# fanzhongyi/ExploreMultiModal

Hardware: AMD Instinct MI355X
Metric: image-text pairs/sec fwd+bwd, VLMo-Base, 1/2/4/8 MI355X; % bf16 MFMA roofline (higher is better)
Workload: dtype bf16

## Files before the change

exploremultimodal_amd/csrc/gemm_tn.hip:

```cpp
#include "gemm_common.h"
#include <algorithm>
#include <vector>

namespace {

struct GemmTN {
    const void* A;
    const void* B;
    float* C;
    int M, N1, N2, lda, ldb, ldc;
    int kt_per_split, tiles;
    float alpha;
    float* slab;
    int mode;
};
enum { TN_ATOMIC = 0, TN_ACCUM = 1, TN_STORE = 2 };

__device__ __attribute__((aligned(256))) char tn_zero_page[256];

__device__ __forceinline__ int tn_swz(int row) { return ((row & 3) << 2) | ((row >> 2) & 3); }

template <typename T, int BM, int BN, int WM, int WN, bool PP = false>
__device__ __forceinline__ void gemm_tn_body(const GemmTN& p, const int lid) {
    typedef typename Elem<T>::v8 v8;
    typedef typename Elem<T>::v4 v4;
    constexpr int NW = WM * WN;
    constexpr int SROWS = PP ? 32 : 64;
    constexpr int SUB = SROWS * 256;
    constexpr int NSA = BM / 128, NSB = BN / 128;
    constexpr int A_BYTES = NSA * SUB, STAGE = (NSA + NSB) * SUB;
    constexpr int TM = BM / WM / 32, TN = BN / WN / 32;
    constexpr int IPS = SROWS / 4;
    constexpr int IA = NSA * IPS / NW, IB = NSB * IPS / NW;
    static_assert((NSA * IPS) % NW == 0 && (NSB * IPS) % NW == 0, "tile/wave mismatch");
    static_assert(!PP || IA + IB == 4, "slice ring: four DMA instructions per wave and slice");
    extern __shared__ __attribute__((aligned(16))) char smem[];
    const int tid = threadIdx.x, lane = tid & 63;
    const int wave = __builtin_amdgcn_readfirstlane(tid >> 6);
    const int wm = wave / WN, wn = wave % WN;
    const int tiles_n = (p.N2 + BN - 1) / BN;
    const int split = lid / p.tiles, tile = lid - split * p.tiles;
    const int n1_0 = (tile / tiles_n) * BM, n2_0 = (tile % tiles_n) * BN;
    const int nk_total = (p.M + 63) >> 6;
    const int kt0 = split * p.kt_per_split;
    const int kt1 = min(nk_total, kt0 + p.kt_per_split);
    if (kt0 >= kt1) return;

// ... 184 lines not shown
                for (int r = 0; r < 16; ++r) {
                    const int gm = gm0 + (r & 3) + 8 * (r >> 2);
                    if (okn && gm < p.N1) p.C[(size_t)gm * p.ldc + gn] = old[r] + p.alpha * acc[i][j][r];
                }
            }
        return;
    }
#pragma unroll
    for (int i = 0; i < TM; ++i)
#pragma unroll
        for (int j = 0; j < TN; ++j) {
            const int gn = n2_0 + wn * (BN / WN) + j * 32 + l31;
#pragma unroll
            for (int r = 0; r < 16; ++r) {
                const int gm = n1_0 + wm * (BM / WM) + i * 32 + (r & 3) + 8 * (r >> 2) + 4 * h;
                if (gm < p.N1 && gn < p.N2) {
                    float* c = p.C + (size_t)gm * p.ldc + gn;
                    if (p.slab)
                        p.slab[((size_t)split * p.N1 + gm) * p.N2 + gn] = acc[i][j][r];
                    else if (p.mode == TN_STORE)
                        *c = p.alpha * acc[i][j][r];
                    else
                        atomicAdd(c, p.alpha * acc[i][j][r]);
                }
            }
        }
}

template <typename T, int BM, int BN, int WM, int WN, bool PP = false>
__global__ __launch_bounds__(WM * WN * 64, 2) void gemm_tn_kernel(const GemmTN p) {
    gemm_tn_body<T, BM, BN, WM, WN, PP>(p, xcd_remap(blockIdx.x, gridDim.x));
}

constexpr int MAX_TN_PROBS = 16;
constexpr int MAX_TN_ORDER = 1024;
constexpr uint16_t TN_NOP = 0xFFFF;
struct GemmTNMulti {
    int n;
    GemmTN p[MAX_TN_PROBS];
    uint16_t order[MAX_TN_ORDER];
};
template <typename T>
__global__ __launch_bounds__(512, 2) void gemm_tn_multi_kernel(const GemmTNMulti mp) {
    const uint32_t code = mp.order[blockIdx.x];
    if (code == TN_NOP) return;
    int gi = (int)(code >> 12);
    const int lid_in = __builtin_amdgcn_readfirstlane((int)(code & 0xFFFu));
    gi = __builtin_amdgcn_readfirstlane(gi);
    const GemmTN& q = mp.p[gi];
    GemmTN p;
    p.A = uniform_ptr(q.A), p.B = uniform_ptr(q.B), p.C = (float*)uniform_ptr(q.C);
    p.M = __builtin_amdgcn_readfirstlane(q.M), p.N1 = __builtin_amdgcn_readfirstlane(q.N1);
    p.N2 = __builtin_amdgcn_readfirstlane(q.N2), p.lda = __builtin_amdgcn_readfirstlane(q.lda);
    p.ldb = __builtin_amdgcn_readfirstlane(q.ldb), p.ldc = __builtin_amdgcn_readfirstlane(q.ldc);
    p.kt_per_split = __builtin_amdgcn_readfirstlane(q.kt_per_split), p.tiles = __builtin_amdgcn_readfirstlane(q.tiles);
    p.alpha = __builtin_bit_cast(float, __builtin_amdgcn_readfirstlane(__builtin_bit_cast(int, q.alpha)));
    p.slab = nullptr;
    p.mode = __builtin_amdgcn_readfirstlane(q.mode);
    gemm_tn_body<T, 256, 256, 2, 4, true>(p, lid_in);
}

__global__ __launch_bounds__(256) void tn_reduce_kernel(const float* __restrict__ slab, int splits, int N1, int N2,
                                                        float* __restrict__ C, int ldc, float alpha) {
    const int n4 = N2 >> 2;
    const long total = (long)N1 * n4;
    for (long i = (long)blockIdx.x * 256 + threadIdx.x; i < total; i += (long)gridDim.x * 256) {
        const int r = (int)(i / n4), c = (int)(i % n4) * 4;
        f32x4 a = {0.f, 0.f, 0.f, 0.f};
        for (int s2 = 0; s2 < splits; ++s2) a += *(const f32x4*)(slab + ((size_t)s2 * N1 + r) * N2 + c);
        f32x4* o = (f32x4*)(C + (size_t)r * ldc + c);
        *o = *o + alpha * a;
    }
}

struct TnPlan {
    int big, tiles, splits, per;
};
TnPlan tn_plan(int M, int N1, int N2, int splits_req, int force_tile) {
    const int nk = (M + 63) / 64;
    TnPlan pl{};
    const int t256 = ((N1 + 255) / 256) * ((N2 + 255) / 256);
    const int t128 = ((N1 + 127) / 128) * ((N2 + 127) / 128);
    const bool big_ok = N1 >= 256 && N2 >= 256 && nk >= 16 && t256 <= 256;
    pl.big = force_tile == 256 ? 1 : (force_tile == 128 ? 0 : (big_ok && (256 / t256) <= 16 && (256 / t256) >= 1 && nk / (256 / t256) >= 8));
    pl.tiles = pl.big ? t256 : t128;
    int splits = splits_req;
    if (splits <= 0) {
        if (pl.big) {
            splits = 256 / pl.tiles;
        } else {
            splits = 512 / pl.tiles;
            if (splits < 4) splits = 1024 / pl.tiles;
// ... 28 lines not shown
    }
    const TnPlan pl = tn_plan(M, N1, N2, splits, force);
    const bool use_slab = ws && pl.splits > 1 && N2 % 4 == 0 && ldc % 4 == 0 && ws_bytes >= (int64_t)pl.splits * N1 * N2 * 4;
    GemmTN p{A, B, C, M, N1, N2, lda, ldb, ldc, pl.per, pl.tiles, alpha, use_slab ? ws : nullptr, TN_ATOMIC};
    dim3 grid(pl.tiles * pl.splits);
    ProfScope prof(64 + (pl.big ? 8 : 0), 2.0 * M * N1 * N2, stream);
    if (pl.big) {
        constexpr int LDS = 2 * 4 * 64 * 256;
        static DeviceOnce attr;
        if (attr.first()) {
            (void)hipFuncSetAttribute((const void*)gemm_tn_kernel<bf16, 256, 256, 2, 4, true>, hipFuncAttributeMaxDynamicSharedMemorySize, LDS);
            (void)hipFuncSetAttribute((const void*)gemm_tn_kernel<f16, 256, 256, 2, 4, true>, hipFuncAttributeMaxDynamicSharedMemorySize, LDS);
        }
        if (dtype == VLMO_F16)
            hipLaunchKernelGGL((gemm_tn_kernel<f16, 256, 256, 2, 4, true>), grid, dim3(512), LDS, stream, p);
        else
            hipLaunchKernelGGL((gemm_tn_kernel<bf16, 256, 256, 2, 4, true>), grid, dim3(512), LDS, stream, p);
    } else {
        if (dtype == VLMO_F16)
            hipLaunchKernelGGL((gemm_tn_kernel<f16, 128, 128, 2, 2>), grid, dim3(256), 65536, stream, p);
        else
            hipLaunchKernelGGL((gemm_tn_kernel<bf16, 128, 128, 2, 2>), grid, dim3(256), 65536, stream, p);
    }
    VLMO_CHECK_LAUNCH("vlmo_gemm_tn");
    if (use_slab) {
        const long total = (long)N1 * (N2 / 4);
        const int rg = (int)((total + 255) / 256 < 2048 ? (total + 255) / 256 : 2048);
        hipLaunchKernelGGL(tn_reduce_kernel, dim3(rg), dim3(256), 0, stream, ws, pl.splits, N1, N2, C, ldc, alpha);
        VLMO_CHECK_LAUNCH("vlmo_gemm_tn(reduce)");
    }
    return 0;
}

extern "C" int vlmo_gemm_tn_multi(int dtype, const VlmoTnProblem* probs, int n, hipStream_t stream) {
    VLMO_CHECK_ARG(probs && n >= 1, "vlmo_gemm_tn_multi: no problems");
    VLMO_CHECK_ARG(dtype == VLMO_BF16 || dtype == VLMO_F16, "vlmo_gemm_tn_multi: dtype must be bf16 or f16");
    static DeviceOnce attr;
    if (attr.first()) {
        constexpr int LDS = 2 * 4 * 64 * 256;
        (void)hipFuncSetAttribute((const void*)gemm_tn_multi_kernel<bf16>, hipFuncAttributeMaxDynamicSharedMemorySize, LDS);
        (void)hipFuncSetAttribute((const void*)gemm_tn_multi_kernel<f16>, hipFuncAttributeMaxDynamicSharedMemorySize, LDS);
    }
    for (int q0 = 0, nq = 0; q0 < n; q0 += nq) {
        nq = 0;
        for (long tl = 0; q0 + nq < n && nq < MAX_TN_PROBS; ++nq) {
            const VlmoTnProblem& r = probs[q0 + nq];
            const long t = (long)((r.N1 + 255) / 256) * ((r.N2 + 255) / 256);
            if (nq > 0 && tl + t > MAX_TN_ORDER - 64) break;
            tl += t;
        }
        long tiles_all = 0;
        int min_nk = 1 << 30;
        double flops = 0;
        for (int q = 0; q < nq; ++q) {
            const VlmoTnProblem& r = probs[q0 + q];
            VLMO_CHECK_ARG(r.A && r.B && r.C, "vlmo_gemm_tn_multi: null operand in problem %d", q0 + q);
            VLMO_CHECK_ARG(r.M > 0 && r.N1 >= 8 && r.N2 >= 8 && r.N1 % 8 == 0 && r.N2 % 8 == 0 && r.lda % 8 == 0 &&
                               r.ldb % 8 == 0 && r.lda >= r.N1 && r.ldb >= r.N2 && r.ldc >= r.N2,
                           "vlmo_gemm_tn_multi: bad shape in problem %d (M=%d N1=%d N2=%d)", q0 + q, r.M, r.N1, r.N2);
            tiles_all += (long)((r.N1 + 255) / 256) * ((r.N2 + 255) / 256);
            const int nk = (r.M + 63) / 64;
            if (nk < min_nk) min_nk = nk;
            flops += 2.0 * r.M * r.N1 * r.N2;
        }
        int splits = 1;
        if (tiles_all < 192) {
            splits = (int)(256 / tiles_all);
            if (splits > min_nk / 8) splits = min_nk / 8;
            if (splits < 1) splits = 1;
        }
        GemmTNMulti mp{};
        mp.n = nq;
        struct Job {
            uint16_t code;
            int cost;
        };
        std::vector<Job> jobs;
        for (int q = 0; q < nq; ++q) {
            const VlmoTnProblem& r = probs[q0 + q];
            const int tiles = ((r.N1 + 255) / 256) * ((r.N2 + 255) / 256);
            const int nk = (r.M + 63) / 64;
            int sp = splits > nk ? nk : splits;
            const int per = (nk + sp - 1) / sp;
            sp = (nk + per - 1) / per;
            int mode = r.accumulate ? TN_ACCUM : TN_STORE;
            if (sp > 1) {
                mode = TN_ATOMIC;
                if (!r.accumulate) {
                    hipError_t rc = hipMemset2DAsync(r.C, (size_t)r.ldc * 4, 0, (size_t)r.N2 * 4, r.N1, stream);
                    if (rc != hipSuccess) {
                        vlmo_set_error("vlmo_gemm_tn_multi: memset failed: %s", hipGetErrorString(rc));
                        return (int)rc;
                    }
                }
            }
            VLMO_CHECK_ARG(tiles * sp <= 4096, "vlmo_gemm_tn_multi: problem %d has too many tiles", q0 + q);
            mp.p[q] = GemmTN{r.A, r.B, r.C, r.M, r.N1, r.N2, r.lda, r.ldb, r.ldc, per, tiles, r.alpha, nullptr, mode};
            for (int l = 0; l < tiles * sp; ++l) jobs.push_back(Job{(uint16_t)((q << 12) | l), per});
        }
        std::stable_sort(jobs.begin(), jobs.end(), [](const Job& a, const Job& b) { return a.cost > b.cost; });
        std::vector<uint16_t> bins[8];
        for (size_t i = 0; i < jobs.size();) {
            size_t j = i;
            while (j < jobs.size() && jobs[j].cost == jobs[i].cost) ++j;
            const size_t cnt = j - i;
            for (int x = 0; x < 8; ++x)
                for (size_t k = i + cnt * x / 8; k < i + cnt * (x + 1) / 8; ++k) bins[x].push_back(jobs[k].code);
            i = j;
        }
        size_t deepest = 0;
        for (int x = 0; x < 8; ++x) deepest = bins[x].size() > deepest ? bins[x].size() : deepest;
        VLMO_CHECK_ARG(deepest * 8 <= (size_t)MAX_TN_ORDER, "vlmo_gemm_tn_multi: %zu workgroups exceed one launch (pass fewer problems per call)",
                       jobs.size());
        const int t = (int)deepest * 8;
        for (int b = 0; b < t; ++b) {
            const std::vector<uint16_t>& bin = bins[b & 7];
            mp.order[b] = (size_t)(b >> 3) < bin.size() ? bin[b >> 3] : TN_NOP;
        }
        ProfScope prof(73, flops, stream);
        constexpr int LDS = 2 * 4 * 64 * 256;
        if (dtype == VLMO_F16)
            hipLaunchKernelGGL((gemm_tn_multi_kernel<f16>), dim3(t), dim3(512), LDS, stream, mp);
        else
            hipLaunchKernelGGL((gemm_tn_multi_kernel<bf16>), dim3(t), dim3(512), LDS, stream, mp);
        VLMO_CHECK_LAUNCH("vlmo_gemm_tn_multi");
    }
    return 0;
}
```

exploremultimodal_amd/hip.py:

```python
import ctypes
import os

import torch

_HERE = os.path.dirname(os.path.abspath(__file__))
LIB_PATH = os.environ.get('VLMO_HIP_LIB') or os.path.join(_HERE, 'lib', 'libvlmo_hip.so')

BF16, F16, F32 = 0, 1, 2
EPI_BIAS, EPI_BIAS_GELU, EPI_RESID, EPI_DGELU, EPI_F32, EPI_DUAL, EPI_ARGMAX, EPI_CE, EPI_CE_BWD = 0, 1, 2, 3, 4, 5, 6, 7, 8

_vp, _i32, _u32, _u64, _f32, _i64 = (ctypes.c_void_p, ctypes.c_int32, ctypes.c_uint32,
                                     ctypes.c_uint64, ctypes.c_float, ctypes.c_int64)


class Epilogue(ctypes.Structure):
    _fields_ = [('out', _vp), ('out2', _vp), ('bias', _vp), ('gamma', _vp),
                ('resid', _vp), ('row_scale', _vp), ('row_index', _vp), ('aux', _vp),
                ('ldo', _i32), ('ld2', _i32), ('relu', _i32),
                ('drop_thresh', _u32), ('inv_keep', _f32), ('beta', _f32),
                ('seed', _u64), ('colpart', _vp)]


_fp = _vp

# ... 49 lines not shown
                     ctypes.POINTER(Epilogue), _vp],
    'vlmo_gemm_tn': [_i32, _vp, _i32, _vp, _i32, _vp, _i32, _i32, _i32, _i32, _f32, _i32, _vp, _i64, _vp],
    'vlmo_ln_fwd': [_vp, _vp, _vp, _vp, _i32, _vp, _vp, _vp, _i32, _i32, _f32, _vp],
    'vlmo_ln_bwd': [_vp, _i32, _vp, _vp, _vp, _vp, _vp, _vp, _vp, _vp, _vp, _i32, _i32, _vp, _i64, _vp],
    'vlmo_ln_resid_bwd': [_vp, _vp, _vp, _vp, _vp, _vp, _vp, _vp, _vp, _vp, _vp, _vp, _vp, _vp, _vp, _vp, _u32, _f32, _u64,
                          _i32, _i32, _vp, _i64, _vp],
    'vlmo_attn_fwd': [_vp, _vp, _i32, _vp, _vp, _vp, _i32, _i32, _i32, _i32, _f32, _u32, _f32,
                      _u64, _i32, _vp],
    'vlmo_attn_bwd': [_vp, _vp, _vp, _vp, _i32, _vp, _i32, _vp, _vp, _vp, _i32, _i32, _i32, _f32,
                      _u32, _f32, _u64, _i32, _vp],
    'vlmo_resid_bwd': [_vp, _vp, _vp, _vp, _vp, _vp, _vp, _vp, _i32, _i32, _u32, _f32, _u64, _vp, _i64, _vp],
    'vlmo_colsum': [_i32, _vp, _i32, _vp, _i32, _i32, _vp, _i64, _vp],
    'vlmo_cast_weight': [_i32, _vp, _i32, _i32, _vp, _vp, _vp],
    'vlmo_cast_weight_multi': [_i32, _i32, _vp, _vp, _vp, _vp, _vp, _vp],
    'vlmo_patchify': [_vp, _vp, _i32, _i32, _i32, _i32, _i32, _vp],
    'vlmo_embed_img_finish': [_vp, _vp, _vp, _vp, _vp, _vp, _vp, _i32, _i32, _i32, _u32, _f32,
                              _u64, _vp],
    'vlmo_embed_img_bwd': [_vp, _vp, _vp, _vp, _vp, _vp, _vp, _i32, _i32, _i32, _u32, _f32,
                           _u64, _vp],
    'vlmo_embed_txt_fwd': [_vp] * 10 + [_i32, _i32, _i32, _f32, _u32, _f32, _u64, _vp],
    'vlmo_embed_txt_bwd': [_vp] * 11 + [_i32, _i32, _i32, _u32, _f32, _u64, _vp],
    'vlmo_conv2d_nhwc': [_i32, _i32, _vp, _i32, _i32, _i32, _i32, _i32, _vp, _i32, _vp,
                         ctypes.POINTER(Epilogue), _vp],
    'vlmo_dvae_im2col': [_vp, _vp, _i32, _i32, _i32, _i32, _i32, _i32, _vp],
    'vlmo_maxpool2_nhwc': [_vp, _vp, _vp, _i32, _i32, _i32, _i32, _vp],
    'vlmo_argmax_reduce': [_vp, _i32, _vp, _i32, _vp],
    'vlmo_dvae_embed': [_vp, _vp, _vp, _vp, _i32, _i32, _i32, _vp],
    'vlmo_upsample2_nhwc': [_vp, _vp, _i32, _i32, _i32, _i32, _vp],
    'vlmo_dvae_out_head': [_vp, _vp, _vp, _vp, _i32, _i32, _i32, _i32, _i32, _vp],
    'vlmo_ce_reduce': [_vp, _i32, _vp, _i32, _vp, _vp, _vp, _i32, _vp],
    'vlmo_stack_fwd': [ctypes.POINTER(StackDesc), _vp],
    'vlmo_stack_bwd': [ctypes.POINTER(StackDesc), _vp],
    'vlmo_gemm_tn_multi': [_i32, ctypes.POINTER(TnProblem), _i32, _vp],
    'vlmo_colwork_multi': [_i32, ctypes.POINTER(ColJob), _i32, _vp],
    'vlmo_event_create': [ctypes.POINTER(ctypes.c_void_p)],
    'vlmo_event_destroy': [_vp],
    'vlmo_stream_wait_event': [_vp, _vp],
    'vlmo_profile_start': [_i32],
    'vlmo_gemm_nt_grouped': [_i32, _i32, _i32, _i32, _vp, _i32, _vp, _i32, _vp, _i32, _i32, _vp, _vp],
    'vlmo_mt_grad_norm': [ctypes.c_void_p, _f32, _f32, _vp, _vp, _vp],
    'vlmo_mt_adam': [ctypes.c_void_p, ctypes.c_void_p, _vp, _vp],
    'vlmo_mt_ema': [ctypes.c_void_p, _f32, _vp],
    'vlmo_mt_adam_ema': [ctypes.c_void_p, ctypes.c_void_p, _vp, _vp, _f32, _vp],
    'vlmo_side_stream_create': [_i32, ctypes.POINTER(ctypes.c_uint32), _i32, ctypes.POINTER(ctypes.c_void_p)],
    'vlmo_profile_stop': [_i32, ctypes.POINTER(ctypes.c_double), ctypes.POINTER(ctypes.c_double),
                          ctypes.POINTER(ctypes.c_int64)],
    'vlmo_gemm_nt_2src': [_i32, _i32, _i32, _vp, _i32, _i32, _f32, _vp, _i32, _vp, _i32, _i32, _i32, _i32,
                          ctypes.POINTER(Epilogue), _vp],
    'vlmo_comm_available': [],
    'vlmo_comm_unique_id': [_vp],
    'vlmo_comm_init': [ctypes.POINTER(ctypes.c_void_p), _vp, _i32, _i32],
    'vlmo_comm_destroy': [_vp],
    'vlmo_comm_count': [_vp, _vp, _vp],
    'vlmo_comm_all_reduce': [_vp, _vp, _vp, _i64, _i32, _vp],
    'vlmo_comm_reduce_scatter': [_vp, _vp, _vp, _i64, _i32, _vp],
    'vlmo_comm_all_gather': [_vp, _vp, _vp, _i64, _i32, _vp],
    'vlmo_grad_pack': [_vp, _vp, _i64, _f32, _vp],
    'vlmo_grad_unpack': [_vp, _vp, _i64, _vp],
    'vlmo_ln_gelu_fwd': [_vp, _i32, _vp, _vp, _vp, _i32, _vp, _vp, _i32, _i32, _f32, _vp],
    'vlmo_ln_gelu_bwd': [_vp, _i32, _vp, _i32, _vp, _vp, _vp, _vp, _vp, _i32, _vp, _i32, _vp, _vp, _vp, _i32, _i32, _vp,
                         _i64, _vp],
    'vlmo_vqa_bce': [_vp, _i32, _vp, _i32, _i32, _i32, _vp, _vp, _vp, _vp, _f32, _vp, _i32, _vp, _i32, _vp],
    'vlmo_isda_update': [_vp, _i32, _vp, _vp, _vp, _vp, _vp, _i32, _i32, _i32, _i32, _vp, _vp, _vp, _vp, _vp],
    'vlmo_isda_aug_fwd': [_vp, _i32, _vp, _vp, _i32, _i32, _i32, _i32, _f32, _vp, _i32, _vp, _i64, _vp],
    'vlmo_isda_aug_bwd': [_vp, _i32, _vp, _i32, _vp, _vp, _i32, _i32, _i32, _i32, _f32, _vp, _i32, _vp, _i64, _vp],
    'vlmo_sim_topk': [_vp, _i32, _vp, _i32, _i32, _i32, _i32, _i32, _f32, _i32, _vp, ctypes.c_size_t, _vp, _vp, _vp],
# ... 265 lines not shown


def maxpool2_nhwc(x, raw, relu, B, H, W, C):
    _check(lib().vlmo_maxpool2_nhwc(_p(x), _p(raw), _p(relu), B, H, W, C, _stream()), 'vlmo_maxpool2_nhwc')


def argmax_reduce(partial, nchunk, ids, M):
    _check(lib().vlmo_argmax_reduce(_p(partial), nchunk, _p(ids), M, _stream()), 'vlmo_argmax_reduce')


def dvae_embed(ids, table, bias, out):
    vocab, n_init = table.shape
    _check(lib().vlmo_dvae_embed(_p(ids), _p(table), _p(bias), _p(out), ids.numel(), vocab, n_init, _stream()),
           'vlmo_dvae_embed')


def upsample2_nhwc(x, out, B, H, W, C):
    _check(lib().vlmo_upsample2_nhwc(_p(x), _p(out), B, H, W, C, _stream()), 'vlmo_upsample2_nhwc')


def dvae_out_head(x, w, bias, out, B, H, W):
    Cout, C = w.shape
    _check(lib().vlmo_dvae_out_head(_p(x), _p(w), _p(bias), _p(out), B, H, W, C, Cout, _stream()), 'vlmo_dvae_out_head')


def gemm_tn_multi(problems, dtype=BF16):
    n = len(problems)
    arr = (TnProblem * n)()
    for i, (A, B, C, M, N1, N2, acc) in enumerate(problems):
        arr[i] = TnProblem(_p(A), _p(B), _p(C), A.stride(0), B.stride(0), C.stride(0), M, N1, N2, 1.0, int(acc))
    _check(lib().vlmo_gemm_tn_multi(dtype, arr, n, _stream()), 'vlmo_gemm_tn_multi')


def colwork_multi(jobs, dtype=BF16):
    n = len(jobs)
    arr = (ColJob * n)()
    for i, (kind, src, rows, ncols, outs, n0) in enumerate(jobs):
        o = (ctypes.c_void_p * 4)(*[_p(t) for t in (list(outs) + [None] * 4)[:4]])
        arr[i] = ColJob(kind, src.stride(0), _p(src), rows, ncols, o, n0, 0)
    _check(lib().vlmo_colwork_multi(dtype, arr, n, _stream()), 'vlmo_colwork_multi')


def event_create():
    out = ctypes.c_void_p()
    _check(lib().vlmo_event_create(ctypes.byref(out)), 'vlmo_event_create')
    return out.value


def stream_wait_event(stream, ev):
    raw = stream.cuda_stream if hasattr(stream, 'cuda_stream') else stream
    _check(lib().vlmo_stream_wait_event(raw, ev), 'vlmo_stream_wait_event')


COMM_ID_BYTES = 128


def comm_available():
    return bool(lib().vlmo_comm_available())


def comm_unique_id():
    buf = ctypes.create_string_buffer(COMM_ID_BYTES)
    _check(lib().vlmo_comm_unique_id(buf), 'vlmo_comm_unique_id')
    return buf.raw


# ... 243 lines not shown
```

include/vlmo_hip.h:

```cpp
#ifndef VLMO_HIP_H
#define VLMO_HIP_H

#include <stddef.h>
#include <stdint.h>

#ifdef __cplusplus
extern "C" {
#endif

#ifndef __HIP_PLATFORM_AMD__
typedef struct ihipStream_t* hipStream_t;
#endif

enum { VLMO_BF16 = 0, VLMO_F16 = 1, VLMO_F32 = 2 };

enum {
    VLMO_EPI_BIAS = 0,
    VLMO_EPI_BIAS_GELU = 1,
    VLMO_EPI_RESID = 2,
    VLMO_EPI_DGELU = 3,
    VLMO_EPI_F32 = 4,
    VLMO_EPI_DUAL = 5,
    VLMO_EPI_ARGMAX = 6,
    VLMO_EPI_CE = 7,
// ... 16 lines not shown
    float beta;
    uint64_t seed;
    float* colpart;
} VlmoEpilogue;

const char* vlmo_last_error(void);
#define VLMO_ABI_VERSION 9
int vlmo_abi_version(void);

int vlmo_gemm_nt(int epi, int dtype, int tile, const void* A, int lda, const void* B, int ldb,
                 int M, int N, int K, const VlmoEpilogue* e, hipStream_t stream);
int vlmo_gemm_nt_2src(int epi, int dtype, int tile, const void* A, int lda, int k1, float seg_scale, const void* A2,
                      int lda2, const void* B, int ldb, int M, int N, int K, const VlmoEpilogue* e,
                      hipStream_t stream);
int vlmo_gemm_nt_grouped(int epi, int dtype, int tile, int ngroups, const void* const* A, int lda,
                         const void* const* B, int ldb, const int32_t* M, int N, int K,
                         const VlmoEpilogue* e, hipStream_t stream);

int64_t vlmo_gemm_tn_ws_bytes(int M, int N1, int N2);
int vlmo_gemm_tn(int dtype, const void* A, int lda, const void* B, int ldb, float* C, int ldc,
                 int M, int N1, int N2, float alpha, int splits, float* ws, int64_t ws_bytes,
                 hipStream_t stream);

typedef struct VlmoTnProblem {
    const void* A;
    const void* B;
    float* C;
    int32_t lda, ldb, ldc;
    int32_t M, N1, N2;
    float alpha;
    int32_t accumulate;
} VlmoTnProblem;
int vlmo_gemm_tn_multi(int dtype, const VlmoTnProblem* probs, int n, hipStream_t stream);

int vlmo_ln_fwd(const float* x, const float* w, const float* b, void* y, int out_f32,
                float* mean, float* rstd, const int32_t* rowmap, int M, int d, float eps,
                hipStream_t stream);
int64_t vlmo_reduce_ws_bytes(int ncols);

int vlmo_ln_bwd(const void* dy, int dy_f32, const int32_t* rowmap, const float* x, const float* w,
                const float* mean, const float* rstd, const float* dres, float* dx, float* dw,
                float* db, int M, int d, float* ws, int64_t ws_bytes, hipStream_t stream);

int vlmo_ln_resid_bwd(const void* dy, const float* x, const float* w, const float* mean, const float* rstd,
                      const float* dres, float* dx, float* dw, float* db, const void* zd, const float* gamma,
                      const float* row_scale, const int32_t* row_index, void* dz, float* dgamma, float* dbias,
                      uint32_t drop_thresh, float inv_keep, uint64_t seed, int M, int d, float* ws,
                      int64_t ws_bytes, hipStream_t stream);

int vlmo_attn_fwd(const void* qkv, const int32_t* seg, int num_seq, const int32_t* keymask,
                  void* ctx, float* lse, int lse_stride, int heads, int d, int max_len,
                  float scale, uint32_t drop_thresh, float inv_keep, uint64_t seed, int mask_seq0,
                  hipStream_t stream);
int vlmo_attn_bwd(const void* qkv, const void* ctx, const void* dctx, const float* lse,
                  int lse_stride, const int32_t* seg, int num_seq, const int32_t* keymask,
                  void* dqkv, float* qv_colsum, int heads, int d, int max_len, float scale,
                  uint32_t drop_thresh, float inv_keep, uint64_t seed, int mask_seq0, hipStream_t stream);

int vlmo_resid_bwd(const float* dx, const void* zd, const float* gamma, const float* row_scale,
                   const int32_t* row_index, void* dz, float* dgamma, float* dbias, int M, int d,
                   uint32_t drop_thresh,
                   float inv_keep, uint64_t seed, float* ws, int64_t ws_bytes, hipStream_t stream);

int vlmo_colsum(int dtype, const void* x, int ld, float* out, int M, int N, float* ws,
                int64_t ws_bytes, hipStream_t stream);

// ... 194 lines not shown
```

Measured before the change: 4520.

## Add variable-height TN GEMM tiles with makespan-planned height and transpose selection

Adds a bf16 TN GEMM body whose tile height is a multiple of 16 rows (192 to 256). It can also compute the transposed product, storing C with vectorized column writes. A host-side planner searches per-shape height/transpose combinations, scores each with a simulated makespan across the eight XCDs and their CUs, and caches the chosen plan. This is meant to reduce tile-quantization waste and load imbalance in the grouped weight-gradient launch. The cost is more host planning work, extra template instantiations with register pressure, and a single-buffered-per-wave 4-slot ring pipeline whose correctness is harder to check.

```diff
diff --git a/exploremultimodal_amd/csrc/gemm_tn.hip b/exploremultimodal_amd/csrc/gemm_tn.hip
--- a/exploremultimodal_amd/csrc/gemm_tn.hip
+++ b/exploremultimodal_amd/csrc/gemm_tn.hip
@@ -1,5 +1,8 @@
 #include "gemm_common.h"
 #include <algorithm>
+#include <cstring>
+#include <mutex>
+#include <type_traits>
 #include <vector>
 
 namespace {
@@ -13,6 +16,7 @@
     float alpha;
     float* slab;
     int mode;
+    int h16, tr;
 };
 enum { TN_ATOMIC = 0, TN_ACCUM = 1, TN_STORE = 2 };
 
@@ -263,6 +267,217 @@
     gemm_tn_body<T, BM, BN, WM, WN, PP>(p, xcd_remap(blockIdx.x, gridDim.x));
 }
 
+template <typename T, int H16>
+__device__ __forceinline__ void gemm_tn16_body(const GemmTN& p, const int lid) {
+    typedef typename Elem<T>::v8 v8;
+    typedef typename Elem<T>::v4 v4;
+    constexpr int TMA = (H16 + 1) / 2, TMB = H16 / 2;
+    constexpr int BM = 16 * H16, BN = 256, WN = 4, NW = 8;
+    constexpr int SROWS = 32, SUB = SROWS * 256, A_BYTES = 2 * SUB, STAGE = 4 * SUB;
+    constexpr int IPS = SROWS / 4, IA = 2 * IPS / NW, IB = IA;
+    static_assert(H16 >= 9 && H16 <= 16, "two sub-images of A, at most eight tile rows per wave group");
+    static_assert(IA + IB == 4, "slice ring: four DMA instructions per wave and slice");
+    extern __shared__ __attribute__((aligned(16))) char smem[];
+    const int tid = threadIdx.x, lane = tid & 63;
+    const int wave = __builtin_amdgcn_readfirstlane(tid >> 6);
+    const int wm = wave / WN, wn = wave % WN;
+    const int tiles_n = (p.N2 + BN - 1) / BN;
+    const int split = lid / p.tiles, tile = lid - split * p.tiles;
+    const int n1_0 = (tile / tiles_n) * BM, n2_0 = (tile % tiles_n) * BN;
+    const int nk_total = (p.M + 63) >> 6;
+    const int kt0 = split * p.kt_per_split;
+    const int kt1 = min(nk_total, kt0 + p.kt_per_split);
+    if (kt0 >= kt1) return;
+
+    int a_off[IA], b_off[IB], a_row[IA], b_row[IB];
+#pragma unroll
+    for (int i = 0; i < IA; ++i) {
+        const int ii = i * NW + wave, sub = ii / IPS, row = (ii % IPS) * 4 + (lane >> 4);
+        const int ch = (lane & 15) ^ tn_swz(row);
+        a_row[i] = b_row[i] = row;
+        a_off[i] = min(n1_0 + sub * 128 + ch * 8, p.N1 - 8);
+        b_off[i] = min(n2_0 + sub * 128 + ch * 8, p.N2 - 8);
+    }
+    const bool fits32 = (uint64_t)p.M * (uint64_t)max(p.lda, p.ldb) * 2 < 0x7FFFFFFFull;
+    BufSrc a_rs, b_rs;
+    a_rs.init(p.A);
+    b_rs.init(p.B);
+    uint32_t a_vo[IA], b_vo[IB];
+#pragma unroll
+    for (int i = 0; i < IA; ++i) {
+        a_vo[i] = (uint32_t)(a_row[i] * p.lda + a_off[i]) * 2u;
+        b_vo[i] = (uint32_t)(b_row[i] * p.ldb + b_off[i]) * 2u;
+    }
+    auto stage = [&](int buf, int kt) {
+        char* s = smem + buf * STAGE;
+        if (fits32 && (kt + 1) * SROWS <= p.M) {
+            const int sa = kt * SROWS * p.lda * 2, sb = kt * SROWS * p.ldb * 2;
+#pragma unroll
+            for (int i = 0; i < IA; ++i) a_rs.load16(s + (i * NW + wave) * 1024, a_vo[i], sa);
+#pragma unroll
+            for (int i = 0; i < IB; ++i) b_rs.load16(s + A_BYTES + (i * NW + wave) * 1024, b_vo[i], sb);
+            return;
+        }
+#pragma unroll
+        for (int i = 0; i < IA; ++i) {
+            const int gr = kt * SROWS + a_row[i];
+            const T* src = gr < p.M ? (const T*)p.A + (size_t)gr * p.lda + a_off[i] : (const T*)tn_zero_page;
+            glds16(src, s + (i * NW + wave) * 1024);
+        }
+#pragma unroll
+        for (int i = 0; i < IB; ++i) {
+            const int gr = min(kt * SROWS + b_row[i], p.M - 1);
+            glds16((const T*)p.B + (size_t)gr * p.ldb + b_off[i], s + A_BYTES + (i * NW + wave) * 1024);
+        }
+    };
+
+    auto body = [&](auto tm_c, const int row0) __attribute__((always_inline)) {
+        constexpr int TM = decltype(tm_c)::value;
+        f32x4 acc[TM][4];
+#pragma unroll
+        for (int i = 0; i < TM; ++i)
+#pragma unroll
+            for (int j = 0; j < 4; ++j) acc[i][j] = f32x4{0.f, 0.f, 0.f, 0.f};
+        const int g = lane >> 4, q = (lane >> 2) & 3, pp = lane & 3, l15 = lane & 15;
+        const uint32_t lds0 = (uint32_t)(uintptr_t)LDS_PTR(smem);
+        uint32_t a_rd[2][TM], b_rd[2][4];
+#pragma unroll
+        for (int half = 0; half < 2; ++half) {
+            const int m0 = 8 * g + 4 * half + q;
+            const int sw = tn_swz(m0);
+#pragma unroll
+            for (int t = 0; t < TM; ++t) {
+                const int na = row0 + t * 16 + 4 * pp;
+                a_rd[half][t] = lds0 + (na >> 7) * SUB + m0 * 256 + ((((na & 127) >> 3) ^ sw) << 4) + (na & 7) * 2;
+            }
+#pragma unroll
+            for (int t = 0; t < 4; ++t) {
+                const int nb = wn * 64 + t * 16 + 4 * pp;
+                b_rd[half][t] = lds0 + A_BYTES + (nb >> 7) * SUB + m0 * 256 + ((((nb & 127) >> 3) ^ sw) << 4) + (nb & 7) * 2;
+            }
+        }
+        v8 af[TM], bf[4];
+        typedef __attribute__((ext_vector_type(2))) uint32_t u32x2;
+        auto tr = [&](uint32_t addr) -> v4 {
+            u32x2 r;
+            asm volatile("ds_read_b64_tr_b16 %0, %1" : "=v"(r) : "v"(addr));
+            return __builtin_bit_cast(v4, r);
+        };
+        auto read_slice = [&](int slot) {
+            const uint32_t so = (uint32_t)slot * STAGE;
+#pragma unroll
+            for (int half = 0; half < 2; ++half) {
+#pragma unroll
+                for (int t = 0; t < 4; ++t) {
+                    const v4 vb = tr(b_rd[half][t] + so);
+#pragma unroll
+                    for (int e = 0; e < 4; ++e) bf[t][4 * half + e] = vb[e];
+                }
+#pragma unroll
+                for (int t = 0; t < TM; ++t) {
+                    const v4 va = tr(a_rd[half][t] + so);
+#pragma unroll
+                    for (int e = 0; e < 4; ++e) af[t][4 * half + e] = va[e];
+                }
+            }
+        };
+        auto mfma_slice = [&]() {
+            __builtin_amdgcn_s_setprio(1);
+#pragma unroll
+            for (int i = 0; i < TM; ++i)
+#pragma unroll
+                for (int j = 0; j < 4; ++j) acc[i][j] = Elem<T>::mfma16(af[i], bf[j], acc[i][j]);
+            __builtin_amdgcn_s_setprio(0);
+        };
+        auto bar = [&]() {
+            __builtin_amdgcn_sched_barrier(0);
+            asm volatile("s_waitcnt lgkmcnt(0)" ::: "memory");
+            __builtin_amdgcn_s_barrier();
+            asm volatile("" ::: "memory");
+            __builtin_amdgcn_sched_barrier(0);
+        };
+        const int ns = 2 * (kt1 - kt0), s0 = 2 * kt0;
+        auto wait_next = [&](int h) {
+            if (h + 3 < ns) asm volatile("s_waitcnt vmcnt(8)" ::: "memory");
+            else if (h + 2 < ns) asm volatile("s_waitcnt vmcnt(4)" ::: "memory");
+            else asm volatile("s_waitcnt vmcnt(0)" ::: "memory");
+        };
+        stage(0, s0);
+        stage(1, s0 + 1);
+        if (ns > 2) stage(2, s0 + 2);
+        wait_next(-1);
+        __builtin_amdgcn_s_barrier();
+        if (wm == 1) bar();
+        for (int h_ = 0; h_ < ns; ++h_) {
+            read_slice(h_ & 3);
+            if (h_ + 3 < ns) stage((h_ + 3) & 3, s0 + h_ + 3);
+            if (wm == 1 && h_ + 1 < ns) wait_next(h_);
+            bar();
+            mfma_slice();
+            if (wm == 0 && h_ + 1 < ns) wait_next(h_);
+            bar();
+        }
+        if (wm == 0) bar();
+
+        const int mode = p.mode;
+#pragma unroll
+        for (int i = 0; i < TM; ++i) {
+            const int gm0 = n1_0 + row0 + i * 16 + 4 * g;
+            if (gm0 >= p.N1) continue;
+            if (p.tr) {
+                f32x4 old[4];
+#pragma unroll
+                for (int j = 0; j < 4; ++j) {
+                    const int gn = n2_0 + wn * 64 + j * 16 + l15;
+                    old[j] = (mode == TN_ACCUM && gn < p.N2) ? *(const f32x4*)(p.C + (size_t)gn * p.ldc + gm0) : f32x4{0.f, 0.f, 0.f, 0.f};
+                }
+#pragma unroll
+                for (int j = 0; j < 4; ++j) {
+                    const int gn = n2_0 + wn * 64 + j * 16 + l15;
+                    if (gn >= p.N2) continue;
+                    float* c = p.C + (size_t)gn * p.ldc + gm0;
+                    if (mode == TN_ATOMIC) {
+#pragma unroll
+                        for (int r = 0; r < 4; ++r) atomicAdd(c + r, p.alpha * acc[i][j][r]);
+                    } else {
+                        *(f32x4*)c = mode == TN_STORE ? p.alpha * acc[i][j] : old[j] + p.alpha * acc[i][j];
+                    }
+                }
+            } else {
+                float old[4][4];
+#pragma unroll
+                for (int j = 0; j < 4; ++j) {
+                    const int gn = n2_0 + wn * 64 + j * 16 + l15;
+#pragma unroll
+                    for (int r = 0; r < 4; ++r)
+                        old[j][r] = (mode == TN_ACCUM && gn < p.N2) ? p.C[(size_t)(gm0 + r) * p.ldc + gn] : 0.f;
+                }
+#pragma unroll
+                for (int j = 0; j < 4; ++j) {
+                    const int gn = n2_0 + wn * 64 + j * 16 + l15;
+                    if (gn >= p.N2) continue;
+#pragma unroll
+                    for (int r = 0; r < 4; ++r) {
+                        float* c = p.C + (size_t)(gm0 + r) * p.ldc + gn;
+                        if (mode == TN_ATOMIC)
+                            atomicAdd(c, p.alpha * acc[i][j][r]);
+                        else
+                            *c = mode == TN_STORE ? p.alpha * acc[i][j][r] : old[j][r] + p.alpha * acc[i][j][r];
+                    }
+                }
+            }
+        }
+    };
+    if constexpr (TMA == TMB) {
+        body(std::integral_constant<int, TMA>{}, wm * 16 * TMA);
+    } else {
+        if (wm == 0)
+            body(std::integral_constant<int, TMA>{}, 0);
+        else
+            body(std::integral_constant<int, TMB>{}, 16 * TMA);
+    }
+}
+
 constexpr int MAX_TN_PROBS = 16;
 constexpr int MAX_TN_ORDER = 1024;
 constexpr uint16_t TN_NOP = 0xFFFF;
@@ -288,7 +503,18 @@
     p.alpha = __builtin_bit_cast(float, __builtin_amdgcn_readfirstlane(__builtin_bit_cast(int, q.alpha)));
     p.slab = nullptr;
     p.mode = __builtin_amdgcn_readfirstlane(q.mode);
-    gemm_tn_body<T, 256, 256, 2, 4, true>(p, lid_in);
+    p.h16 = __builtin_amdgcn_readfirstlane(q.h16), p.tr = __builtin_amdgcn_readfirstlane(q.tr);
+    if constexpr (std::is_same<T, bf16>::value) {
+        switch (p.h16) {
+            case 12: gemm_tn16_body<T, 12>(p, lid_in); break;
+            case 13: gemm_tn16_body<T, 13>(p, lid_in); break;
+            case 14: gemm_tn16_body<T, 14>(p, lid_in); break;
+            case 15: gemm_tn16_body<T, 15>(p, lid_in); break;
+            default: gemm_tn16_body<T, 16>(p, lid_in); break;
+        }
+    } else {
+        gemm_tn_body<T, 256, 256, 2, 4, true>(p, lid_in);
+    }
 }
 
 __global__ __launch_bounds__(256) void tn_reduce_kernel(const float* __restrict__ slab, int splits, int N1, int N2,
@@ -383,98 +609,315 @@
     return 0;
 }
 
-extern "C" int vlmo_gemm_tn_multi(int dtype, const VlmoTnProblem* probs, int n, hipStream_t stream) {
+namespace {
+constexpr double TN_COST_C = 1.0;
+constexpr int TN_H16_MIN = 12, TN_H16_MAX = 16;
+constexpr int TN_PLAN_MAX_SHAPES = 6, TN_PLAN_MAX_COMBOS = 40000;
+
+struct TnOpt {
+    int h16, tr, tiles;
+};
+int tn_tiles(const VlmoTnProblem& r, int h16, int tr) {
+    const int ns = tr ? r.N2 : r.N1, nl = tr ? r.N1 : r.N2;
+    return ((ns + 16 * h16 - 1) / (16 * h16)) * ((nl + 255) / 256);
+}
+bool tn_tr_ok(const VlmoTnProblem& r) { return r.ldc % 4 == 0 && ((uintptr_t)r.C & 15) == 0; }
+
+void tn_class_runs(int cnt, int& rot, int out[8]) {
+    const int base = cnt / 8, rem = cnt % 8;
+    for (int x = 0; x < 8; ++x) out[x] = base + (((x - rot) & 7) < rem ? 1 : 0);
+    rot = (rot + rem) & 7;
+}
+struct TnClass {
+    double cost;
+    int cnt;
+};
+double tn_makespan(const std::vector<TnClass>& cls) {
+    double worst = 0;
+    std::vector<int> runs(cls.size() * 8);
+    int rot = 0;
+    for (size_t c = 0; c < cls.size(); ++c) tn_class_runs(cls[c].cnt, rot, &runs[c * 8]);
+    for (int x = 0; x < 8; ++x) {
+        double cu[32] = {0};
+        for (size_t c = 0; c < cls.size(); ++c)
+            for (int k = 0; k < runs[c * 8 + x]; ++k) {
+                int best = 0;
+                for (int u = 1; u < 32; ++u)
+                    if (cu[u] < cu[best]) best = u;
+                cu[best] += cls[c].cost;
+            }
+        for (int u = 0; u < 32; ++u) worst = cu[u] > worst ? cu[u] : worst;
+    }
+    return worst;
+}
+double tn_cost(int per, int h16) { return per * (h16 + TN_COST_C); }
+double tn_makespan_of(const VlmoTnProblem* probs, int nq, const TnOpt* ch) {
+    std::vector<TnClass> cls;
+    for (int q = 0; q < nq; ++q) {
+        const double c = tn_cost((probs[q].M + 63) / 64, ch[q].h16);
+        size_t k = 0;
+        while (k < cls.size() && cls[k].cost != c) ++k;
+        if (k == cls.size()) cls.push_back(TnClass{c, 0});
+        cls[k].cnt += ch[q].tiles;
+    }
+    std::sort(cls.begin(), cls.end(), [](const TnClass& a, const TnClass& b) { return a.cost > b.cost; });
+    return tn_makespan(cls);
+}
+
+void tn_plan_heights(const VlmoTnProblem* probs, int nq, const int* forced, TnOpt* out) {
+    struct Key {
+        int v[MAX_TN_PROBS][5];
+        int nq;
+    };
+    struct Entry {
+        Key k;
+        TnOpt o[MAX_TN_PROBS];
+    };
+    static std::mutex mu;
+    static std::vector<Entry> cache;
+    Key key{};
+    key.nq = nq;
+    for (int q = 0; q < nq; ++q) {
+        const VlmoTnProblem& r = probs[q];
+        const int kv[5] = {r.M, r.N1, r.N2, forced ? forced[q] : 0, tn_tr_ok(r) ? 1 : 0};
+        for (int i = 0; i < 5; ++i) key.v[q][i] = kv[i];
+    }
+    std::lock_guard<std::mutex> lock(mu);
+    for (const Entry& e : cache)
+        if (memcmp(&e.k, &key, sizeof(Key)) == 0) {
+            for (int q = 0; q < nq; ++q) out[q] = e.o[q];
+            return;
+        }
+    int shape_of[MAX_TN_PROBS], ns = 0, rep[MAX_TN_PROBS];
+    for (int q = 0; q < nq; ++q) {
+        int s2 = 0;
+        while (s2 < ns && memcmp(key.v[rep[s2]], key.v[q], sizeof(key.v[q])) != 0) ++s2;
+        if (s2 == ns) rep[ns++] = q;
+        shape_of[q] = s2;
+    }
+    std::vector<std::vector<TnOpt>> opts(ns);
+    long combos = 1;
+    for (int s2 = 0; s2 < ns; ++s2) {
+        const VlmoTnProblem& r = probs[rep[s2]];
+        const int f = key.v[rep[s2]][3];
+        if (f) {
+            opts[s2].push_back(TnOpt{f < 0 ? -f : f, f < 0, tn_tiles(r, f < 0 ? -f : f, f < 0)});
+            continue;
+        }
+        std::vector<TnOpt> all;
+        for (int h = TN_H16_MAX; h >= TN_H16_MIN; --h)
+            for (int tr = 0; tr < (tn_tr_ok(r) ? 2 : 1); ++tr) all.push_back(TnOpt{h, tr, tn_tiles(r, h, tr)});
+        for (size_t a = 0; a < all.size(); ++a) {
+            bool dominated = false;
+            for (size_t b = 0; b < all.size() && !dominated; ++b) {
+                if (b == a || all[b].h16 > all[a].h16 || all[b].tiles > all[a].tiles) continue;
+                dominated = all[b].h16 < all[a].h16 || all[b].tiles < all[a].tiles || b < a;
+            }
+            if (!dominated) opts[s2].push_back(all[a]);
+        }
+        combos *= (long)opts[s2].size();
+    }
+    std::vector<int> idx(ns, 0), best_idx(ns, 0);
+    TnOpt cur[MAX_TN_PROBS];
+    auto fill = [&](const std::vector<int>& ix) {
+        for (int q = 0; q < nq; ++q) cur[q] = opts[shape_of[q]][ix[shape_of[q]]];
+    };
+    fill(idx);
+    double best = tn_makespan_of(probs, nq, cur);
+    if (ns <= TN_PLAN_MAX_SHAPES && combos <= TN_PLAN_MAX_COMBOS) {
+        for (;;) {
+            int d = 0;
+            while (d < ns && ++idx[d] == (int)opts[d].size()) idx[d++] = 0;
+            if (d == ns) break;
+            fill(idx);
+            long jobs = 0;
+            double total = 0, longest = 0;
+            for (int q = 0; q < nq; ++q) {
+                const double c = tn_cost((probs[q].M + 63) / 64, cur[q].h16);
+                jobs += cur[q].tiles;
+                total += c * cur[q].tiles;
+                longest = c > longest ? c : longest;
+            }
+            if (jobs > MAX_TN_ORDER - 16) continue;
+            if (longest >= best || total / 256 >= best) continue;
+            const double m = tn_makespan_of(probs, nq, cur);
+            if (m < best * (1 - 1e-9)) best = m, best_idx = idx;
+        }
+    }
+    fill(best_idx);
+    Entry e{};
+    e.k = key;
+    for (int q = 0; q < nq; ++q) out[q] = e.o[q] = cur[q];
+    if (cache.size() >= 64) cache.erase(cache.begin());
+    cache.push_back(e);
+}
+
+struct TnLaunch {
+    int nq, t;
+    double flops, makespan, makespan256;
+    GemmTNMulti mp;
+    bool clear[MAX_TN_PROBS];
+};
+int tn_multi_prepare(const VlmoTnProblem* probs, int n, const int* h16, int force_splits, TnLaunch& L) {
+    auto tiles_hint = [&](int q) {
+        const VlmoTnProblem& r = probs[q];
+        const int f = h16 ? h16[q] : 0;
+        return (long)(f ? tn_tiles(r, f < 0 ? -f : f, f < 0) : tn_tiles(r, 16, 0));
+    };
+    int nq = 0;
+    for (long tl = 0; nq < n && nq < MAX_TN_PROBS; ++nq) {
+        const long t = tiles_hint(nq);
+        if (nq > 0 && tl + t > MAX_TN_ORDER - 64) break;
+        tl += t;
+    }
+    L.nq = nq;
+    long tiles_all = 0;
+    int min_nk = 1 << 30;
+    L.flops = 0;
+    for (int q = 0; q < nq; ++q) {
+        const VlmoTnProblem& r = probs[q];
+        VLMO_CHECK_ARG(r.M > 0 && r.N1 >= 8 && r.N2 >= 8 && r.N1 % 8 == 0 && r.N2 % 8 == 0 && r.lda % 8 == 0 &&
+                           r.ldb % 8 == 0 && r.lda >= r.N1 && r.ldb >= r.N2 && r.ldc >= r.N2,
+                       "vlmo_gemm_tn_multi: bad shape in problem %d (M=%d N1=%d N2=%d)", q, r.M, r.N1, r.N2);
+        const int f = h16 ? h16[q] : 0, fa = f < 0 ? -f : f;
+        VLMO_CHECK_ARG(f == 0 || (fa >= TN_H16_MIN && fa <= TN_H16_MAX), "vlmo_gemm_tn_multi: tile height %d of problem %d outside %d..%d",
+                       f, q, TN_H16_MIN, TN_H16_MAX);
+        VLMO_CHECK_ARG(f >= 0 || tn_tr_ok(r), "vlmo_gemm_tn_multi: problem %d cannot be written transposed (ldc %% 4, alignment of C)", q);
+        tiles_all += tn_tiles(r, 16, 0);
+        const int nk = (r.M + 63) / 64;
+        if (nk < min_nk) min_nk = nk;
+        L.flops += 2.0 * r.M * r.N1 * r.N2;
+    }
+    int splits = 1;
+    if (force_splits > 0) {
+        splits = force_splits;
+    } else if (tiles_all < 192) {
+        splits = (int)(256 / tiles_all);
+        if (splits > min_nk / 8) splits = min_nk / 8;
+        if (splits < 1) splits = 1;
+    }
+    TnOpt ch[MAX_TN_PROBS], ch256[MAX_TN_PROBS];
+    for (int q = 0; q < nq; ++q) {
+        const int f = h16 ? h16[q] : 0, fa = f < 0 ? -f : f;
+        ch256[q] = TnOpt{16, 0, tn_tiles(probs[q], 16, 0)};
+        ch[q] = f ? TnOpt{fa, f < 0, tn_tiles(probs[q], fa, f < 0)} : ch256[q];
+    }
+    if (splits == 1) tn_plan_heights(probs, nq, h16, ch);
+    L.makespan = tn_makespan_of(probs, nq, ch);
+    L.makespan256 = tn_makespan_of(probs, nq, ch256);
+
+    L.mp = GemmTNMulti{};
+    L.mp.n = nq;
+    struct Job {
+        uint16_t code;
+        double cost;
+    };
+    std::vector<Job> jobs;
+    for (int q = 0; q < nq; ++q) {
+        const VlmoTnProblem& r = probs[q];
+        const int tiles = ch[q].tiles;
+        const int nk = (r.M + 63) / 64;
+        int sp = splits > nk ? nk : splits;
+        const int per = (nk + sp - 1) / sp;
+        sp = (nk + per - 1) / per;
+        int mode = r.accumulate ? TN_ACCUM : TN_STORE;
+        L.clear[q] = false;
+        if (sp > 1 || force_splits > 1) {
+            mode = TN_ATOMIC;
+            L.clear[q] = !r.accumulate;
+        }
+        VLMO_CHECK_ARG(tiles * sp <= 4096, "vlmo_gemm_tn_multi: problem %d has too many tiles", q);
+        GemmTN& g = L.mp.p[q];
+        g = GemmTN{r.A, r.B, r.C, r.M, r.N1, r.N2, r.lda, r.ldb, r.ldc, per, tiles, r.alpha, nullptr, mode, ch[q].h16, ch[q].tr};
+        if (ch[q].tr) {
+            g.A = r.B, g.B = r.A, g.N1 = r.N2, g.N2 = r.N1, g.lda = r.ldb, g.ldb = r.lda;
+        }
+        for (int l = 0; l < tiles * sp; ++l) jobs.push_back(Job{(uint16_t)((q << 12) | l), tn_cost(per, ch[q].h16)});
+    }
+    std::stable_sort(jobs.begin(), jobs.end(), [](const Job& a, const Job& b) { return a.cost > b.cost; });
+    std::vector<uint16_t> bins[8];
+    int rot = 0;
+    for (size_t i = 0; i < jobs.size();) {
+        size_t j = i;
+        while (j < jobs.size() && jobs[j].cost == jobs[i].cost) ++j;
+        int runs[8];
+        tn_class_runs((int)(j - i), rot, runs);
+        size_t k = i;
+        for (int x = 0; x < 8; ++x)
+            for (int e = 0; e < runs[x]; ++e) bins[x].push_back(jobs[k++].code);
+        i = j;
+    }
+    size_t deepest = 0;
+    for (int x = 0; x < 8; ++x) deepest = bins[x].size() > deepest ? bins[x].size() : deepest;
+    VLMO_CHECK_ARG(deepest * 8 <= (size_t)MAX_TN_ORDER, "vlmo_gemm_tn_multi: %zu workgroups exceed one launch (pass fewer problems per call)",
+                   jobs.size());
+    L.t = (int)deepest * 8;
+    for (int b = 0; b < L.t; ++b) {
+        const std::vector<uint16_t>& bin = bins[b & 7];
+        L.mp.order[b] = (size_t)(b >> 3) < bin.size() ? bin[b >> 3] : TN_NOP;
+    }
+    return 0;
+}
+
+int tn_multi_run(int dtype, const VlmoTnProblem* probs, int n, const int* h16, int force_splits, hipStream_t stream) {
     VLMO_CHECK_ARG(probs && n >= 1, "vlmo_gemm_tn_multi: no problems");
     VLMO_CHECK_ARG(dtype == VLMO_BF16 || dtype == VLMO_F16, "vlmo_gemm_tn_multi: dtype must be bf16 or f16");
+    VLMO_CHECK_ARG(force_splits >= 0 && force_splits <= 16, "vlmo_gemm_tn_multi: splits must be 0..16 (got %d)", force_splits);
+    if (dtype == VLMO_F16 && h16)
+        for (int q = 0; q < n; ++q) VLMO_CHECK_ARG(h16[q] == 0, "vlmo_gemm_tn_multi: f16 runs 256-row tiles only");
+    constexpr int LDS = 2 * 4 * 64 * 256;
     static DeviceOnce attr;
     if (attr.first()) {
-        constexpr int LDS = 2 * 4 * 64 * 256;
         (void)hipFuncSetAttribute((const void*)gemm_tn_multi_kernel<bf16>, hipFuncAttributeMaxDynamicSharedMemorySize, LDS);
         (void)hipFuncSetAttribute((const void*)gemm_tn_multi_kernel<f16>, hipFuncAttributeMaxDynamicSharedMemorySize, LDS);
     }
-    for (int q0 = 0, nq = 0; q0 < n; q0 += nq) {
-        nq = 0;
-        for (long tl = 0; q0 + nq < n && nq < MAX_TN_PROBS; ++nq) {
-            const VlmoTnProblem& r = probs[q0 + nq];
-            const long t = (long)((r.N1 + 255) / 256) * ((r.N2 + 255) / 256);
-            if (nq > 0 && tl + t > MAX_TN_ORDER - 64) break;
-            tl += t;
-        }
-        long tiles_all = 0;
-        int min_nk = 1 << 30;
-        double flops = 0;
-        for (int q = 0; q < nq; ++q) {
+    static const int pin256[MAX_TN_PROBS] = {16, 16, 16, 16, 16, 16, 16, 16, 16, 16, 16, 16, 16, 16, 16, 16};
+    TnLaunch L;
+    for (int q0 = 0; q0 < n; q0 += L.nq) {
+        for (int q = q0; q < n && q < q0 + MAX_TN_PROBS; ++q)
+            VLMO_CHECK_ARG(probs[q].A && probs[q].B && probs[q].C, "vlmo_gemm_tn_multi: null operand in problem %d", q);
+        const int rc0 = tn_multi_prepare(probs + q0, n - q0, dtype == VLMO_F16 ? pin256 : (h16 ? h16 + q0 : nullptr), force_splits, L);
+        if (rc0) return rc0;
+        for (int q = 0; q < L.nq; ++q) {
+            if (!L.clear[q]) continue;
             const VlmoTnProblem& r = probs[q0 + q];
-            VLMO_CHECK_ARG(r.A && r.B && r.C, "vlmo_gemm_tn_multi: null operand in problem %d", q0 + q);
-            VLMO_CHECK_ARG(r.M > 0 && r.N1 >= 8 && r.N2 >= 8 && r.N1 % 8 == 0 && r.N2 % 8 == 0 && r.lda % 8 == 0 &&
-                               r.ldb % 8 == 0 && r.lda >= r.N1 && r.ldb >= r.N2 && r.ldc >= r.N2,
-                           "vlmo_gemm_tn_multi: bad shape in problem %d (M=%d N1=%d N2=%d)", q0 + q, r.M, r.N1, r.N2);
-            tiles_all += (long)((r.N1 + 255) / 256) * ((r.N2 + 255) / 256);
-            const int nk = (r.M + 63) / 64;
-            if (nk < min_nk) min_nk = nk;
-            flops += 2.0 * r.M * r.N1 * r.N2;
-        }
-        int splits = 1;
-        if (tiles_all < 192) {
-            splits = (int)(256 / tiles_all);
-            if (splits > min_nk / 8) splits = min_nk / 8;
-            if (splits < 1) splits = 1;
-        }
-        GemmTNMulti mp{};
-        mp.n = nq;
-        struct Job {
-            uint16_t code;
-            int cost;
-        };
-        std::vector<Job> jobs;
-        for (int q = 0; q < nq; ++q) {
-            const VlmoTnProblem& r = probs[q0 + q];
-            const int tiles = ((r.N1 + 255) / 256) * ((r.N2 + 255) / 256);
-            const int nk = (r.M + 63) / 64;
-            int sp = splits > nk ? nk : splits;
-            const int per = (nk + sp - 1) / sp;
-            sp = (nk + per - 1) / per;
-            int mode = r.accumulate ? TN_ACCUM : TN_STORE;
-            if (sp > 1) {
-                mode = TN_ATOMIC;
-                if (!r.accumulate) {
-                    hipError_t rc = hipMemset2DAsync(r.C, (size_t)r.ldc * 4, 0, (size_t)r.N2 * 4, r.N1, stream);
-                    if (rc != hipSuccess) {
-                        vlmo_set_error("vlmo_gemm_tn_multi: memset failed: %s", hipGetErrorString(rc));
-                        return (int)rc;
-                    }
-                }
-            }
-            VLMO_CHECK_ARG(tiles * sp <= 4096, "vlmo_gemm_tn_multi: problem %d has too many tiles", q0 + q);
-            mp.p[q] = GemmTN{r.A, r.B, r.C, r.M, r.N1, r.N2, r.lda, r.ldb, r.ldc, per, tiles, r.alpha, nullptr, mode};
-            for (int l = 0; l < tiles * sp; ++l) jobs.push_back(Job{(uint16_t)((q << 12) | l), per});
-        }
-        std::stable_sort(jobs.begin(), jobs.end(), [](const Job& a, const Job& b) { return a.cost > b.cost; });
-        std::vector<uint16_t> bins[8];
-        for (size_t i = 0; i < jobs.size();) {
-            size_t j = i;
-            while (j < jobs.size() && jobs[j].cost == jobs[i].cost) ++j;
-            const size_t cnt = j - i;
-            for (int x = 0; x < 8; ++x)
-                for (size_t k = i + cnt * x / 8; k < i + cnt * (x + 1) / 8; ++k) bins[x].push_back(jobs[k].code);
-            i = j;
-        }
-        size_t deepest = 0;
-        for (int x = 0; x < 8; ++x) deepest = bins[x].size() > deepest ? bins[x].size() : deepest;
-        VLMO_CHECK_ARG(deepest * 8 <= (size_t)MAX_TN_ORDER, "vlmo_gemm_tn_multi: %zu workgroups exceed one launch (pass fewer problems per call)",
-                       jobs.size());
-        const int t = (int)deepest * 8;
-        for (int b = 0; b < t; ++b) {
-            const std::vector<uint16_t>& bin = bins[b & 7];
-            mp.order[b] = (size_t)(b >> 3) < bin.size() ? bin[b >> 3] : TN_NOP;
-        }
-        ProfScope prof(73, flops, stream);
-        constexpr int LDS = 2 * 4 * 64 * 256;
+            hipError_t rc = hipMemset2DAsync(r.C, (size_t)r.ldc * 4, 0, (size_t)r.N2 * 4, r.N1, stream);
+            if (rc != hipSuccess) {
+                vlmo_set_error("vlmo_gemm_tn_multi: memset failed: %s", hipGetErrorString(rc));
+                return (int)rc;
+            }
+        }
+        ProfScope prof(73, L.flops, stream);
         if (dtype == VLMO_F16)
-            hipLaunchKernelGGL((gemm_tn_multi_kernel<f16>), dim3(t), dim3(512), LDS, stream, mp);
+            hipLaunchKernelGGL((gemm_tn_multi_kernel<f16>), dim3(L.t), dim3(512), LDS, stream, L.mp);
         else
-            hipLaunchKernelGGL((gemm_tn_multi_kernel<bf16>), dim3(t), dim3(512), LDS, stream, mp);
+            hipLaunchKernelGGL((gemm_tn_multi_kernel<bf16>), dim3(L.t), dim3(512), LDS, stream, L.mp);
         VLMO_CHECK_LAUNCH("vlmo_gemm_tn_multi");
     }
     return 0;
 }
+}
+
+extern "C" int vlmo_gemm_tn_multi(int dtype, const VlmoTnProblem* probs, int n, hipStream_t stream) {
+    return tn_multi_run(dtype, probs, n, nullptr, 0, stream);
+}
+
+extern "C" int vlmo_gemm_tn_multi_h(int dtype, const VlmoTnProblem* probs, int n, const int* h16, int splits, hipStream_t stream) {
+    return tn_multi_run(dtype, probs, n, h16, splits, stream);
+}
+
+extern "C" int vlmo_gemm_tn_multi_plan(const VlmoTnProblem* probs, int n, const int* h16, int* h16_out, uint16_t* order_out,
+                                       int order_cap, int* order_len, double* makespan, double* makespan256) {
+    VLMO_CHECK_ARG(probs && n >= 1 && h16_out && order_len && makespan && makespan256, "vlmo_gemm_tn_multi_plan: null argument");
+    TnLaunch L;
+    const int rc = tn_multi_prepare(probs, n, h16, 0, L);
+    if (rc) return rc;
+    VLMO_CHECK_ARG(L.nq == n, "vlmo_gemm_tn_multi_plan: the list needs more than one launch (%d of %d problems fit)", L.nq, n);
+    VLMO_CHECK_ARG(!order_out || order_cap >= L.t, "vlmo_gemm_tn_multi_plan: order_out holds %d entries, %d needed", order_cap, L.t);
+    for (int q = 0; q < n; ++q) h16_out[q] = L.mp.p[q].tr ? -L.mp.p[q].h16 : L.mp.p[q].h16;
+    for (int b = 0; order_out && b < L.t; ++b) order_out[b] = L.mp.order[b];
+    *order_len = L.t;
+    *makespan = L.makespan;
+    *makespan256 = L.makespan256;
+    return 0;
+}
diff --git a/exploremultimodal_amd/hip.py b/exploremultimodal_amd/hip.py
--- a/exploremultimodal_amd/hip.py
+++ b/exploremultimodal_amd/hip.py
@@ -105,6 +105,10 @@
     'vlmo_stack_fwd': [ctypes.POINTER(StackDesc), _vp],
     'vlmo_stack_bwd': [ctypes.POINTER(StackDesc), _vp],
     'vlmo_gemm_tn_multi': [_i32, ctypes.POINTER(TnProblem), _i32, _vp],
+    'vlmo_gemm_tn_multi_h': [_i32, ctypes.POINTER(TnProblem), _i32, ctypes.POINTER(_i32), _i32, _vp],
+    'vlmo_gemm_tn_multi_plan': [ctypes.POINTER(TnProblem), _i32, ctypes.POINTER(_i32), ctypes.POINTER(_i32),
+                                ctypes.POINTER(ctypes.c_uint16), _i32, ctypes.POINTER(_i32),
+                                ctypes.POINTER(ctypes.c_double), ctypes.POINTER(ctypes.c_double)],
     'vlmo_colwork_multi': [_i32, ctypes.POINTER(ColJob), _i32, _vp],
     'vlmo_event_create': [ctypes.POINTER(ctypes.c_void_p)],
     'vlmo_event_destroy': [_vp],
@@ -436,6 +440,29 @@
     _check(lib().vlmo_gemm_tn_multi(dtype, arr, n, _stream()), 'vlmo_gemm_tn_multi')
 
 
+def gemm_tn_multi_h(problems, h16, splits=0, dtype=BF16):
+    n = len(problems)
+    arr = (TnProblem * n)()
+    for i, (A, B, C, M, N1, N2, acc) in enumerate(problems):
+        arr[i] = TnProblem(_p(A), _p(B), _p(C), A.stride(0), B.stride(0), C.stride(0), M, N1, N2, 1.0, int(acc))
+    hs = (_i32 * n)(*[int(h) for h in h16])
+    _check(lib().vlmo_gemm_tn_multi_h(dtype, arr, n, hs, splits, _stream()), 'vlmo_gemm_tn_multi_h')
+
+
+def gemm_tn_multi_plan(shapes, h16=None):
+    n = len(shapes)
+    arr = (TnProblem * n)()
+    for i, (M, N1, N2) in enumerate(shapes):
+        arr[i] = TnProblem(256, 256, 256, N1, N2, N2, M, N1, N2, 1.0, 0)
+    hs = (_i32 * n)(*[int(h) for h in (h16 or [0] * n)])
+    out = (_i32 * n)()
+    order = (ctypes.c_uint16 * 1024)()
+    olen, ms, ms256 = _i32(0), ctypes.c_double(0), ctypes.c_double(0)
+    _check(lib().vlmo_gemm_tn_multi_plan(arr, n, hs, out, order, 1024, ctypes.byref(olen), ctypes.byref(ms),
+                                         ctypes.byref(ms256)), 'vlmo_gemm_tn_multi_plan')
+    return list(out), list(order[:olen.value]), ms.value, ms256.value
+
+
 def colwork_multi(jobs, dtype=BF16):
     n = len(jobs)
     arr = (ColJob * n)()
diff --git a/include/vlmo_hip.h b/include/vlmo_hip.h
--- a/include/vlmo_hip.h
+++ b/include/vlmo_hip.h
@@ -72,6 +72,9 @@
     int32_t accumulate;
 } VlmoTnProblem;
 int vlmo_gemm_tn_multi(int dtype, const VlmoTnProblem* probs, int n, hipStream_t stream);
+int vlmo_gemm_tn_multi_h(int dtype, const VlmoTnProblem* probs, int n, const int* h16, int splits, hipStream_t stream);
+int vlmo_gemm_tn_multi_plan(const VlmoTnProblem* probs, int n, const int* h16, int* h16_out, uint16_t* order_out,
+                            int order_cap, int* order_len, double* makespan, double* makespan256);
 
 int vlmo_ln_fwd(const float* x, const float* w, const float* b, void* y, int out_f32,
                 float* mean, float* rstd, const int32_t* rowmap, int M, int d, float eps,
```

Result: slower. 4473 (-1.1%).
